# deveshjawla/MuZero.jl

Hardware: AMD Instinct MI355X
Metric: self-play MCTS node-expansions/sec + train steps/sec, TicTacToe FC net, 1-8 GPU (higher is better)
Workload: dtype f32; 1 GPU; TicTacToe FC (params.jl hyper), 512 games/GPU x 50 sims/move (configs[1]); games_per_gpu=512, sims_per_move=50, global_games=512, parallelism=games sharded x1

## Files before the change

muzero.jl_amd/csrc/mz_small.hip:

```cpp
#include "mz_mlp_device.h"
#include "mz_tree_device.h"

#include "mz_small_params.h"
#include "mz_replay_device.h"
#include "mz_learner_device.h"

#ifdef MZ_STAMPS
#define SM_STAMP(i)                                                              \
    do {                                                                         \
        if (threadIdx.x == 0) {                                                  \
            unsigned long long t_ = __builtin_amdgcn_s_memtime();                \
            st_acc[i] += t_ - st_last; st_last = t_;                             \
        }                                                                        \
    } while (0)
#define W_STAMP0() unsigned long long w_t0_ = __builtin_amdgcn_s_memtime()
#define W_STAMP(k) do { w_acc[k] += __builtin_amdgcn_s_memtime() - w_t0_; } while (0)
#else
#define SM_STAMP(i) do {} while (0)
#define W_STAMP0() do {} while (0)
#define W_STAMP(k) do {} while (0)
#endif

__device__ __forceinline__ int sm_slot_row(int tid) {
    return (tid >> 8) * 64 + ((tid >> 6) & 3) * 16 + (tid & 15);
}

template <int J>
__device__ __forceinline__ void fmac_bcast(float& acc, float x, float w) {
    asm volatile("v_fmac_f32_dpp %0, %1, %2 row_newbcast:%3 row_mask:0xf bank_mask:0xf"
                 : "+v"(acc) : "v"(x), "v"(w), "i"(J));
}

#define SM_F2(j, wj)                                                                              \
    "v_fmac_f32_dpp %0, %2, " wj " row_newbcast:" #j " row_mask:0xf bank_mask:0xf\n\t"            \
    "v_fmac_f32_dpp %1, %3, " wj " row_newbcast:" #j " row_mask:0xf bank_mask:0xf\n\t"

template <int T, int J = 0>
__device__ __forceinline__ void sm_chain(const float (&w)[16], const float (&x)[T], float (&acc)[T]) {
    if constexpr (T == 2 && J == 0) {
        asm volatile("s_nop 1\n\t"
                     SM_F2(0, "%4") SM_F2(1, "%5") SM_F2(2, "%6") SM_F2(3, "%7")
                     SM_F2(4, "%8") SM_F2(5, "%9") SM_F2(6, "%10") SM_F2(7, "%11")
                     SM_F2(8, "%12") SM_F2(9, "%13") SM_F2(10, "%14") SM_F2(11, "%15")
                     SM_F2(12, "%16") SM_F2(13, "%17") SM_F2(14, "%18") SM_F2(15, "%19")
                     : "+v"(acc[0]), "+v"(acc[1])
                     : "v"(x[0]), "v"(x[1]), "v"(w[0]), "v"(w[1]), "v"(w[2]), "v"(w[3]), "v"(w[4]), "v"(w[5]),
                       "v"(w[6]), "v"(w[7]), "v"(w[8]), "v"(w[9]), "v"(w[10]), "v"(w[11]), "v"(w[12]), "v"(w[13]),
                       "v"(w[14]), "v"(w[15]));
    } else if constexpr (J < 16) {
#pragma unroll
        for (int g = 0; g < T; ++g) fmac_bcast<J>(acc[g], x[g], w[J]);
        sm_chain<T, J + 1>(w, x, acc);
    }
}

struct SmFusedIn {
    const float* hid; const int* leaf_e; const int* leaf_a; const float* aval;
    int NN, H, plane, x_pred, x_dyn;
};

template <int T>
__device__ __forceinline__ int sm_xoff(int4 R) {
    const int q = (threadIdx.x >> 4) & 3, i = threadIdx.x & 15;
    return (R.x + ((int)__umul24((unsigned)q, (unsigned)R.y) + i) * T) * 4;
}

template <int T, int FI = 0, int BNM = 1>
__device__ __forceinline__ int4 sm_stage(const float (&w)[16], int4 R, int& xo, const int4* rec_next, float* lds,
                                         const SmFusedIn* fi = nullptr, const float2* bnp = nullptr) {
    const int q = (threadIdx.x >> 4) & 3;
    const float* xp = reinterpret_cast<const float*>(reinterpret_cast<const char*>(lds) + xo);
    float x[T];
    if constexpr (FI != 0) {
        const int k = (int)__umul24((unsigned)q, (unsigned)R.y) + (int)(threadIdx.x & 15);
        const bool pred = R.x == fi->x_pred, dyn = R.x == fi->x_dyn;
#pragma unroll
        for (int g = 0; g < T; ++g) {
            float hv, av;
            if constexpr (FI == 1) {
                const float* hp = fi->hid + ((size_t)g * fi->NN + fi->leaf_e[g]) * fi->H;
                hv = k < fi->H ? hp[k] : 0.0f;
                av = fi->aval[fi->leaf_a[g]];
            } else {
                hv = k < fi->H ? fi->hid[k * T + g] : 0.0f;
                av = fi->aval[g * fi->NN];
            }
            x[g] = pred ? hv : dyn ? (k < fi->H ? hv * 2.0f : k < fi->H + fi->plane ? av : 0.0f) : xp[g];
        }
    } else if constexpr (T == 1) {
        x[0] = xp[0];
    } else if constexpr (T == 2) {
        const float2 v = *reinterpret_cast<const float2*>(xp);
        x[0] = v.x; x[1] = v.y;
    } else {
        const float4 v = *reinterpret_cast<const float4*>(xp);
        x[0] = v.x; x[1] = v.y; x[2] = v.z; x[3] = v.w;
    }
    const int4 Rn = *rec_next;
    float acc[T];
#pragma unroll
    for (int g = 0; g < T; ++g) acc[g] = 0.0f;
    sm_chain<T>(w, x, acc);
#pragma unroll
    for (int g = 0; g < T; ++g) {
        const auto s1 = __builtin_amdgcn_permlane16_swap(__builtin_bit_cast(unsigned, acc[g]),
                                                         __builtin_bit_cast(unsigned, acc[g]), false, false);
        const float t = __builtin_bit_cast(float, (unsigned)s1[0]) + __builtin_bit_cast(float, (unsigned)s1[1]);
        const auto s2 = __builtin_amdgcn_permlane32_swap(__builtin_bit_cast(unsigned, t),
                                                         __builtin_bit_cast(unsigned, t), false, false);
        acc[g] = __builtin_bit_cast(float, (unsigned)s2[0]) + __builtin_bit_cast(float, (unsigned)s2[1]);
    }
    if (q < T && R.z >= 0) {
        float v = acc[0];
#pragma unroll
        for (int g = 1; g < T; ++g) v = q == g ? acc[g] : v;
        const int o = R.z & 0x1fffffff;
        float d = v + __int_as_float(R.w);
        if constexpr (BNM != 0)
            if ((R.z >> 29) & 1) { const float2 gb = *bnp; d = mz_bn_apply(d, gb.x, gb.y); }
        lds[o + q] = (R.z >> 30) != 0 ? mz_relu(d) : d;
    }
    xo = sm_xoff<T>(Rn);
    asm volatile("" : "+v"(xo));
    __syncthreads();
    return Rn;
}

template <int T, int NMAX, int FI, int OFF, int BNM, int K = 0>
__device__ __forceinline__ void sm_run_k(int n, const float (&wr)[NMAX][16], int4 R, int xo, const int4* rec,
                                         float* lds, const SmFusedIn* fi, const float2* bnp) {
    if constexpr (K + OFF < NMAX) {
        if (K < n) {
            const float2* bk = bnp + K * (SM_SLOTS * 64);
            const int4 Rn = K == 0 && FI != 0
                ? sm_stage<T, FI, BNM>(wr[K + OFF], R, xo, rec + (K + 1) * (SM_SLOTS * 64), lds, fi, bk)
                : sm_stage<T, 0, BNM>(wr[K + OFF], R, xo, rec + (K + 1) * (SM_SLOTS * 64), lds, nullptr, bk);
            sm_run_k<T, NMAX, FI, OFF, BNM, K + 1>(n, wr, Rn, xo, rec, lds, fi, bnp);
        }
    }
}

template <int T, int NMAX, int FI = 0, int OFF = 0, int BNM = 1>
__device__ __forceinline__ void sm_run(int n, const float (&wr)[NMAX][16], const int4* rec, float* lds,
                                       const SmFusedIn* fi, const float2* bnp) {
    const int4 R0 = rec[0];
    sm_run_k<T, NMAX, FI, OFF, BNM>(n, wr, R0, sm_xoff<T>(R0), rec, lds, fi, bnp);
}

template <int NMAX, int DST = 0>
__device__ __forceinline__ void sm_load(int k0, int k1, const float* W, float (&wr)[NMAX][16], const uint32_t* nzm,
                                        const float4* zero16) {
    const int tid = threadIdx.x, sl = tid >> 8, t = tid & 255, q = (tid >> 4) & 3;
    const int w = __builtin_amdgcn_readfirstlane(tid >> 6);
    uint32_t mk[NMAX - DST];
#pragma unroll
    for (int k = 0; k < NMAX - DST; ++k) mk[k] = nzm[w * SM_NZM_ST + k];
#pragma unroll
    for (int k = 0; k < NMAX - DST; ++k) {
        if (k >= k0 && k < k1) {
            const float4* src = reinterpret_cast<const float4*>(W + (((size_t)k * SM_SLOTS + sl) * 4) * 1024) + t;
            const uint32_t m = mk[k] >> (4 * q);
#pragma unroll
            for (int i = 0; i < 4; ++i) {
                const float4 v = *((m >> i) & 1u ? src + i * 256 : zero16);
                wr[k + DST][4 * i] = v.x; wr[k + DST][4 * i + 1] = v.y; wr[k + DST][4 * i + 2] = v.z;
                wr[k + DST][4 * i + 3] = v.w;
            }
        }
    }
}

template <int T, int BNM>
__device__ __forceinline__ void small_body(const SmallParams& P) {
#ifdef MZ_STAMPS
    unsigned long long st_acc[8] = {0, 0, 0, 0, 0, 0, 0, 0};
    unsigned long long st_last = __builtin_amdgcn_s_memtime();
    unsigned long long w_acc[3] = {0, 0, 0};
#endif
    extern __shared__ __attribute__((aligned(16))) float smem[];
    const int A = P.A, S = P.S, H = P.H;
    const int E = (S + 1) * A, NN = S + 1;
    const int PS = 2 * (S + 2);
    const int nrec = P.n_sim + P.n_root;
    float* act = smem;
    int* rec = reinterpret_cast<int*>(act + P.act_total);
    float* hid = reinterpret_cast<float*>(rec + (nrec + 1) * SM_REC_INTS);
    int* si = reinterpret_cast<int*>(hid + ((size_t)T * NN * H + 3) / 4 * 4);
    uint32_t* sg_legal = reinterpret_cast<uint32_t*>(si);
    int* sg_root_tp = si + 16;
    int* sg_rootN = si + 32;
    float* sg_rootW = reinterpret_cast<float*>(si + 48);
    float* sg_mmin = reinterpret_cast<float*>(si + 64);
    float* sg_mmax = reinterpret_cast<float*>(si + 80);
    int* sg_leaf_e = si + 96;
    int* sg_leaf_a = si + 112;
    int* sg_vtp = si + 128;
    int* sg_depth = si + 144;
    float* sg_stage = reinterpret_cast<float*>(si + 160);
    float* sg_noise = reinterpret_cast<float*>(si + 232);
    int* sg_path = si + 296;
    double* l_pbc = reinterpret_cast<double*>(si + 296 + (T * PS + 3) / 4 * 4);
    double* l_sqrt = l_pbc + (S + 2);
    float* l_aval = reinterpret_cast<float*>(l_sqrt + (S + 2));
    double* l_pbterm = reinterpret_cast<double*>(l_aval + MZ_MAX_ACTIONS);
    char* lds_tree = reinterpret_cast<char*>(l_pbterm + pbterm_count(S));
    uint2* c_cache = reinterpret_cast<uint2*>(lds_tree + (size_t)T * P.tree_game_bytes);
    uint2* c_lvl = c_cache + T * NN;
    int* c_nN = reinterpret_cast<int*>(c_lvl + T * (S + 2));
    int4* c_hdr = reinterpret_cast<int4*>(reinterpret_cast<char*>(smem) +
                                          ((reinterpret_cast<char*>(c_nN + T * NN) - reinterpret_cast<char*>(smem) + 15) & ~15));
    float2* c_mmx = reinterpret_cast<float2*>(c_hdr + 4);
    int* c_skip = reinterpret_cast<int*>(c_mmx + 4);
    const bool sel_ballot = NN <= 64;
    const int NNS = sel_ballot ? NN : 0;
    uint4* c_stat = reinterpret_cast<uint4*>(c_skip + 4);
    float2* bnl = reinterpret_cast<float2*>(c_stat + T * NNS);

    const int tid = threadIdx.x;
    const int g = tid >> 4, a = tid & 15, lane = tid & 63;
    const int tile0 = blockIdx.x * T;
    const bool tree_thread = tid < 16 * T;
    const int gg = tile0 + g;
    const bool active = tree_thread && gg < P.G;
    const uint32_t gid = P.game_offset + (uint32_t)gg;
    int* path = sg_path + (tree_thread ? g : 0) * PS;
    TreeView tree = tree_view(lds_tree + (size_t)(tree_thread ? g : 0) * P.tree_game_bytes, E, NN);
    const int4* rec_sim = reinterpret_cast<const int4*>(rec) + sm_slot_row(tid);
    const int4* rec_root = rec_sim + P.n_sim * (SM_SLOTS * 64);
    const float2* bn_sim = bnl + sm_slot_row(tid);
    const float2* bn_root = bn_sim + P.n_sim * (SM_SLOTS * 64);

    float wr[SM_MAX_SIM][16];
    sm_load<SM_MAX_SIM>(0, P.n_root, P.w_root, wr, P.nzm + P.n_sim, P.zero16);
    sm_load<SM_MAX_SIM>(P.n_root, P.n_sim, P.w_sim, wr, P.nzm, P.zero16);
    for (int i = tid; i < P.act_total; i += SM_THREADS) act[i] = 0.0f;
    for (int i = tid; i < S + 2; i += SM_THREADS) { l_pbc[i] = P.pbc_tab[i]; l_sqrt[i] = P.sqrt_tab[i]; }
    if (tid < A) l_aval[tid] = P.aval_tab[tid];
    for (int i = tid; i < (int)pbterm_count(S); i += SM_THREADS) l_pbterm[i] = P.pbterm[i];
    for (int i = tid; i < nrec * SM_REC_INTS; i += SM_THREADS) rec[i] = P.rec[i];
    __syncthreads();
    for (int i = tid; i < nrec * SM_SLOTS * 64; i += SM_THREADS)
        rec[4 * i + 3] = __float_as_int(P.bias[i]);
    if (P.bn)
        for (int i = tid; i < nrec * SM_SLOTS * 64; i += SM_THREADS)
            bnl[i] = make_float2(P.bias[nrec * SM_SLOTS * 64 + i], P.bias[2 * nrec * SM_SLOTS * 64 + i]);
    for (int i = tid; i < T * P.obs_feat; i += SM_THREADS) {
        const int gl = i / P.obs_feat, k = i - gl * P.obs_feat;
        const int ggl = tile0 + gl;
        act[P.x_rep + k * T + gl] = ggl < P.G ? P.obs[(size_t)ggl * P.obs_feat + k] : 0.0f;
    }
    for (int i = tid; i < T * NN; i += SM_THREADS) c_cache[i] = make_uint2(0u, 0u);
    if (tid < 4) { c_hdr[tid] = make_int4(0, -1, 1, 0); c_mmx[tid] = make_float2(0.0f, 0.0f); c_skip[tid] = 0; }
    if (tid < T && sel_ballot) c_stat[tid * NNS] = node_static(0, 0, 0, 1ull);
    int ver = 1;
    if (tree_thread && a == 0) {
        uint32_t m = 0;
        if (active)
            for (int b = 0; b < A; ++b) if (P.legal[(size_t)gg * A + b]) m |= 1u << b;
        sg_legal[g] = m;
        sg_root_tp[g] = active ? P.to_play[gg] : 1;
        sg_rootN[g] = 0; sg_rootW[g] = 0.0f;
        sg_mmin[g] = INFINITY; sg_mmax[g] = -INFINITY;
        sg_leaf_e[g] = 0; sg_leaf_a[g] = 0; sg_vtp[g] = 1; sg_depth[g] = 0;
    }
    __syncthreads();

    if (P.exploration && active)
        sg_noise[16 * g + a] = root_noise_lane(sg_legal[g], a, A, P.seed, gid, P.rng_step, P.dirichlet_alpha,
                                               sg_stage + 16 * g);
    sm_run<T, SM_MAX_SIM, 0, 0, BNM>(P.n_root, wr, rec_root, act, nullptr, bn_root);
    for (int i = tid; i < T * H; i += SM_THREADS) {
        const int gl = i / H, k = i - gl * H;
        const float h = act[P.h_out + k * T + gl];
        hid[(size_t)gl * NN * H + k] = h;
        act[P.x_pred + k * T + gl] = h;
    }
    sm_load<SM_MAX_SIM>(0, P.n_root < P.n_sim ? P.n_root : P.n_sim, P.w_sim, wr, P.nzm, P.zero16);
    __syncthreads();
    sm_run<T, SM_MAX_SIM, 0, 0, BNM>(P.n_sim, wr, rec_sim, act, nullptr, bn_sim);

    const uint32_t legal = tree_thread ? sg_legal[g] : 0u;
    if (tree_thread) {
        const float prior = double_softmax_prior(a < A ? act[P.p_out + a * T + g] : 0.0f, a, A, legal,
                                                 sg_stage + 16 * g);
        if (active) {
            init_edges(tree, 0, a, A, prior);
            if (a == 0) { tree.nr[0] = 0.0f; tree.ntp[0] = (int8_t)sg_root_tp[g]; }
        }
    }
    __syncthreads();
    if (P.exploration && active && a < A && ((legal >> a) & 1u))
        tree.p(a) = tree.p(a) * (1.0f - P.exploration_eps) + sg_noise[16 * g + a] * P.exploration_eps;
    __syncthreads();
    SM_STAMP(0);

    const SmFusedIn fin{hid, sg_leaf_e, sg_leaf_a, l_aval, NN, H, P.plane, P.x_pred, P.x_dyn};
    int n_fast = 0;
    for (int s = 0; s < S; ++s) {
        if (tid < 64 * T) {
            const int w = __builtin_amdgcn_readfirstlane(tid >> 6);
            if (tile0 + w < P.G) {
                const TreeView tw = tree_view(lds_tree + (size_t)w * P.tree_game_bytes, E, NN);
                int* pw = sg_path + w * PS;
                const uint2* cw = c_cache + w * NN;
                const uint32_t verw = (uint32_t)c_hdr[w].z;
                const int rtp = sg_root_tp[w];
                SelectOut so{0, 0, 1, 0};
                int D, e0;
                uint32_t npc0;
                bool found = false;
                if (sel_ballot) {
                    found = select_path_ballot(tw, cw, c_stat + w * NNS, verw, pw, s + 1, s + 1, rtp, lane, A,
                                               P.players, so, D, e0, npc0);
                } else {
                    D = c_skip[w];
                    e0 = D > 0 ? pw[2 * D + 1] : 0;
                    npc0 = D > 0 ? tw.nc(pw[2 * D]) : 0u;
                }
                if (!found && lane < 16) {
                    so = select_path_cached(tw, cw, verw, pw, sg_rootN[w], rtp, sg_legal[w], sg_mmin[w], sg_mmax[w],
                                            lane, lane, A, P.players, l_pbterm, P.seed,
                                            P.game_offset + (uint32_t)(tile0 + w), P.rng_step, s, nullptr, nullptr, D,
                                            e0, npc0);
                    if (sel_ballot && lane == 0) {
                        const uint4 ps = c_stat[w * NNS + so.leaf_e];
                        c_stat[w * NNS + s + 1] = node_static(so.leaf_e, so.depth, so.leaf_a,
                                                              ((uint64_t)ps.y | ((uint64_t)ps.z << 32)) | (1ull << (s + 1)));
                    }
                }
                if (lane == 0) { sg_leaf_e[w] = so.leaf_e; sg_leaf_a[w] = so.leaf_a; sg_vtp[w] = so.vtp; sg_depth[w] = so.depth; }
                n_fast += found ? 1 : 0;
            }
            __builtin_amdgcn_wave_barrier();
            SM_STAMP(1);
        }
        __syncthreads();
#ifdef MZ_STAMPS
        if (threadIdx.x == 0) {
            int md = 0;
            for (int gl = 0; gl < T; ++gl) md = md > sg_depth[gl] ? md : sg_depth[gl];
            st_acc[7] += (unsigned long long)md;
        }
#endif
        SM_STAMP(2);
        sm_run<T, SM_MAX_SIM, 1, 0, BNM>(P.n_sim, wr, rec_sim, act, &fin, bn_sim);
        SM_STAMP(3);
        const int e_new = s + 1;
        if (tid < 64) {
            if (active) {
                const int tl = sg_vtp[g];
                const int depth = sg_depth[g];
                const BackupPre bpre = backup_preload(tree, path, depth, a);
                const bool odd = (a & 1) != 0;
                const float ro = mz_post_act(odd ? P.r_act : P.v_act, act[(odd ? P.r_out : P.v_out) + g]);
                const float val = __builtin_bit_cast(float, __builtin_amdgcn_update_dpp(
                    0, __builtin_bit_cast(int, ro), 0x00, 0xF, 0xF, false));
                const float rew = __builtin_bit_cast(float, __builtin_amdgcn_update_dpp(
                    0, __builtin_bit_cast(int, ro), 0x55, 0xF, 0xF, false));
#ifdef MZ_STAMPS
                if (threadIdx.x == 0) asm volatile("" :: "v"(val), "v"(rew));
#endif
                SM_STAMP(5);
                W_STAMP0();
                if (a == 0) {
                    const int li = sg_leaf_e[g] * A + sg_leaf_a[g];
                    tree.nc(li) = (tree.nc(li) & 0xffffu) | ((uint32_t)(e_new + 1) << 16);
                    tree.nr[e_new] = rew;
                    tree.ntp[e_new] = (int8_t)tl;
                    path[2 * depth + 1] = e_new;
                }
                __builtin_amdgcn_wave_barrier();
                int rN = sg_rootN[g];
                float rW = sg_rootW[g], mmin = sg_mmin[g], mmax = sg_mmax[g];
                const uint32_t omin = __float_as_uint(mmin), omax = __float_as_uint(mmax);
                if (P.players == 2)
                    backup_path_pre(tree, path, bpre, depth, val, rew, e_new, tl, P.discount, rN, rW, sg_root_tp[g],
                                    mmin, mmax, a, c_lvl + g * (S + 2), c_nN + g * NN);
                else
                    backup_path(tree, path, depth, val, tl, A, P.players, P.discount, rN, rW, sg_root_tp[g], mmin,
                                mmax, a, c_lvl + g * (S + 2), c_nN + g * NN);
                const bool moved = __float_as_uint(mmin) != omin || __float_as_uint(mmax) != omax;
                ver += moved ? 1 : 0;
                if (a == 0) {
                    sg_rootN[g] = rN; sg_rootW[g] = rW; sg_mmin[g] = mmin; sg_mmax[g] = mmax;
                    c_hdr[g] = make_int4(moved ? 1 : 0, depth, ver, (int)legal);
                    c_mmx[g] = make_float2(mmin, mmax);
                    c_skip[g] = moved ? 0 : depth;
                }
                W_STAMP(0);
            }
        } else if (tid >= 128 && tid < 128 + 16 * T) {
            W_STAMP0();
            const int g2 = (tid - 128) >> 4;
            const bool active2 = tile0 + g2 < P.G;
            TreeView tree2 = tree_view(lds_tree + (size_t)g2 * P.tree_game_bytes, E, NN);
            const float prior = double_softmax_prior(a < A ? act[P.p_out + a * T + g2] : 0.0f, a, A, sg_legal[g2],
                                                     sg_stage + 16 * g2);
            if (active2) init_edges(tree2, e_new, a, A, prior);
            W_STAMP(1);
        } else if (tid >= 192) {
            W_STAMP0();
            for (int i = tid - 192; i < T * H; i += SM_THREADS - 192) {
                const int gl = i / H, k = i - gl * H;
                hid[((size_t)gl * NN + e_new) * H + k] = act[P.h_out + k * T + gl];
                if (tile0 + gl < P.G) {
                    float* hp = hid + ((size_t)gl * NN + sg_leaf_e[gl]) * H + k;
                    *hp = *hp * 2.0f;
                }
            }
            W_STAMP(2);
        }
        __syncthreads();
        SM_STAMP(4);
        if (s + 1 < S) {
            const int r = tid >> 4, gq = r % T, j0 = r / T;
            int4 hd = c_hdr[gq];
            float2 mm = c_mmx[gq];
            uint2 l0 = c_lvl[gq * (S + 2) + j0];
            int n0 = c_nN[gq * NN + j0];
            asm volatile("" : "+v"(hd.x), "+v"(hd.y), "+v"(hd.z), "+v"(hd.w), "+v"(mm.x), "+v"(mm.y), "+v"(l0.x),
                              "+v"(l0.y), "+v"(n0));
            const bool full = hd.x != 0;
            const int n = full ? s + 2 : hd.y + 1;
            const bool lgl = a < A && (((uint32_t)hd.w >> a) & 1u);
            const TreeView tq = tree_view(lds_tree + (size_t)gq * P.tree_game_bytes, E, NN);
            uint2* cq = c_cache + gq * NN;
            const int* pq = sg_path + gq * PS;
            const int pe0 = !full && j0 < hd.y ? pq[2 * (j0 + 1)] : 0;
            if (j0 < n) {
                const int ch = cache_row(tq, cq, (uint32_t)hd.z, full ? j0 : (int)l0.x, full ? n0 : (int)l0.y, lgl,
                                         a, A, mm.x, mm.y, l_pbterm, lane);
                if (!full && a == 0 && (j0 >= hd.y || ch != pe0 - (int)l0.x * A)) atomicMin(c_skip + gq, j0);
            }
            for (int j = j0 + SM_THREADS / 16 / T; j < n; j += SM_THREADS / 16 / T) {
                int slot, Np;
                if (full) { slot = j; Np = c_nN[gq * NN + j]; }
                else { const uint2 l = c_lvl[gq * (S + 2) + j]; slot = (int)l.x; Np = (int)l.y; }
                const int ch = cache_row(tq, cq, (uint32_t)hd.z, slot, Np, lgl, a, A, mm.x, mm.y, l_pbterm, lane);
                if (!full && a == 0 && (j >= hd.y || ch != pq[2 * (j + 1)] - slot * A)) atomicMin(c_skip + gq, j);
            }
            __syncthreads();
            SM_STAMP(6);
        }
    }
    __syncthreads();

    if (active) {
        const bool lg = a < A && ((legal >> a) & 1u);
        const int Nc = lg ? (int)(tree.nc(a) & 0xffffu) : 0;
        const int sum = g16_isum(Nc);
        if (a < A) P.child_visits[(size_t)gg * A + a] = lg ? (float)((double)Nc / (double)sum) : 0.0f;
        const uint32_t r = mz_rng_u32(P.seed, MZ_RNG_ACTION, gid, P.rng_step, 0);
        const int act = select_action_dev<16>(Nc, legal, A, P.temp_g ? P.temp_g[gg] : P.temperature, r);
        if (a == 0) {
            const int rN = sg_rootN[g];
            P.root_value[gg] = rN == 0 ? 0.0f : sg_rootW[g] / (float)rN;
            P.action_out[gg] = act + 1;
        }
        if (P.dump_tree) {
            TreeView dst = tree_view(P.tree + (size_t)gg * P.tree_game_bytes, E, NN);
            dump_tree(tree, dst, E, NN, a);
        }
    }
    if (P.sel_stats && tid < 64 * T && lane == 0 && tile0 + (tid >> 6) < P.G) {
        P.sel_stats[2 * (tile0 + (tid >> 6))] = n_fast;
        P.sel_stats[2 * (tile0 + (tid >> 6)) + 1] = S - n_fast;
    }
#ifdef MZ_STAMPS
    SM_STAMP(6);
    if (threadIdx.x == 0 && P.stamps)
        for (int i = 0; i < 8; ++i) P.stamps[blockIdx.x * 8 + i] = st_acc[i];
    if (P.stamps && (threadIdx.x == 0 || threadIdx.x == 128 || threadIdx.x == 192)) {
        const int k = threadIdx.x == 0 ? 0 : threadIdx.x == 128 ? 1 : 2;
        P.stamps[(gridDim.x + blockIdx.x) * 8 + k] = w_acc[k];
    }
#endif
}

extern "C" __global__ __launch_bounds__(SM_THREADS, 1) void mz_search_small1(SmallParams P) { small_body<1, 0>(P); }
extern "C" __global__ __launch_bounds__(SM_THREADS, 1) void mz_search_small2(SmallParams P) { small_body<2, 0>(P); }
extern "C" __global__ __launch_bounds__(SM_THREADS, 1) void mz_search_small4(SmallParams P) { small_body<4, 0>(P); }
extern "C" __global__ __launch_bounds__(SM_THREADS, 1) void mz_search_small1_bn(SmallParams P) { small_body<1, 1>(P); }
extern "C" __global__ __launch_bounds__(SM_THREADS, 1) void mz_search_small2_bn(SmallParams P) { small_body<2, 1>(P); }
extern "C" __global__ __launch_bounds__(SM_THREADS, 1) void mz_search_small4_bn(SmallParams P) { small_body<4, 1>(P); }

struct SmIO {
    const float* obs; const float* actions; float* pv; float* pp; float* pr;
    const float* w_sim; const float* w_root; const float* bias;
};
__device__ __forceinline__ SmIO sm_io(const SmallUnrollParams& P) {
    return SmIO{P.obs, P.actions, P.pv, P.pp, P.pr, P.w_sim, P.w_root, P.bias};
}

template <int T, int BNM>
__device__ __forceinline__ void unroll_body(const SmallUnrollParams& P, int lb, const SmIO& io) {
#ifdef MZ_STAMPS
    unsigned long long st_acc[8] = {0, 0, 0, 0, 0, 0, 0, 0};
    unsigned long long st_last = __builtin_amdgcn_s_memtime();
#endif
    extern __shared__ __attribute__((aligned(16))) float smem[];
    const int K = P.K, A = P.A, H = P.H;
    const int nrec = P.n_sim + P.n_root;
    float* act = smem;
    int* rec = reinterpret_cast<int*>(act + P.act_total);
    float* aval = reinterpret_cast<float*>(rec + (nrec + 1) * SM_REC_INTS);
    float2* bnl = reinterpret_cast<float2*>(aval + 64);
    const int tid = threadIdx.x;
    const int tile0 = lb * T;
    const int o_gl = tid / (A + 2), o_c = tid - o_gl * (A + 2);
    const int nri = nrec * SM_SLOTS * 64;
    constexpr int RPT = ((SM_MAX_SIM + SM_MAX_ROOT) * SM_SLOTS * 64 + SM_THREADS - 1) / SM_THREADS;
    const bool sample_first = !P.pf_hdr && P.sample;
    if (sample_first && (tid >> 6) < T && tile0 + (tid >> 6) < P.B) rp_sample_one(P.rp, tile0 + (tid >> 6), tid & 63);
    if (sample_first) { __threadfence_block(); __syncthreads(); }
    long long hd[4] = {0, 0, 0, 0}, cnt0 = 0;
    if (P.pf_hdr) { hd[0] = P.pf_hdr[0]; hd[1] = P.pf_hdr[1]; hd[2] = P.pf_hdr[2]; hd[3] = P.pf_hdr[3]; cnt0 = P.rp.counters[0]; }
    int rx[RPT], ry[RPT], rz[RPT];
    float bv[RPT];
#pragma unroll
    for (int u = 0; u < RPT; ++u) {
        const int i = tid + u * SM_THREADS;
        const int ic = i < nri ? i : 0;
        const int4 r = reinterpret_cast<const int4*>(P.rec)[ic];
        rx[u] = r.x; ry[u] = r.y; rz[u] = r.z;
        bv[u] = io.bias[ic];
    }
    const int o_i = tid / P.obs_feat, o_k = tid - o_i * P.obs_feat;
    const int a_i = tid / (K + 1), a_k = tid - a_i * (K + 1);
    const bool o_in = tid < T * P.obs_feat && tile0 + o_i < P.B, a_in = tid < T * (K + 1) && tile0 + a_i < P.B;
    float ov = o_in ? io.obs[(size_t)(tile0 + o_i) * P.obs_feat + o_k] : 0.0f;
    float av = a_in ? io.actions[(size_t)(tile0 + a_i) * (K + 1) + a_k] : 0.0f;
    float wr[SM_MAX_SIM][16];
    constexpr int RO = SM_MAX_SIM - SM_MAX_ROOT;
    sm_load<SM_MAX_SIM, RO>(0, P.n_root, io.w_root, wr, P.nzm + P.n_sim, P.zero16);
    sm_load<SM_MAX_SIM>(0, RO < P.n_sim ? RO : P.n_sim, io.w_sim, wr, P.nzm, P.zero16);
    sm_load<SM_MAX_SIM>(RO + P.n_root, P.n_sim, io.w_sim, wr, P.nzm, P.zero16);
    const bool have = P.pf_hdr && hd[0] == P.pf_epoch && hd[1] == cnt0 && hd[2] == (long long)P.rp.step &&
                      hd[3] == (long long)P.B;
    if (P.pf_hdr && P.sample && !have) {
        if ((tid >> 6) < T && tile0 + (tid >> 6) < P.B) rp_sample_one(P.rp, tile0 + (tid >> 6), tid & 63);
        __threadfence_block();
        __syncthreads();
        ov = o_in ? io.obs[(size_t)(tile0 + o_i) * P.obs_feat + o_k] : 0.0f;
        av = a_in ? io.actions[(size_t)(tile0 + a_i) * (K + 1) + a_k] : 0.0f;
    }
    for (int i = tid; i < P.act_total; i += SM_THREADS) act[i] = 0.0f;
#pragma unroll
    for (int u = 0; u < RPT; ++u) {
        const int i = tid + u * SM_THREADS;
        if (i < nri) reinterpret_cast<int4*>(rec)[i] = make_int4(rx[u], ry[u], rz[u], __float_as_int(bv[u]));
    }
    if (tid < SM_REC_INTS / 4) reinterpret_cast<int4*>(rec)[nri + tid] = make_int4(0, 0, -1, 0);
    if (P.bn)
        for (int i = tid; i < nri; i += SM_THREADS) bnl[i] = make_float2(io.bias[nri + i], io.bias[2 * nri + i]);
    __syncthreads();
    if (o_in) act[P.x_rep + o_k * T + o_i] = ov;
    if (a_in) aval[a_i * (K + 1) + a_k] = av / (float)A;
    __syncthreads();
    SM_STAMP(0);
    const int4* rec_sim = reinterpret_cast<const int4*>(rec) + sm_slot_row(tid);
    const int4* rec_root = rec_sim + P.n_sim * (SM_SLOTS * 64);
    const float2* bn_sim = bnl + sm_slot_row(tid);
    const float2* bn_root = bn_sim + P.n_sim * (SM_SLOTS * 64);
    sm_run<T, SM_MAX_SIM, 0, RO, BNM>(P.n_root, wr, rec_root, act, nullptr, bn_root);
    SM_STAMP(1);
    sm_load<SM_MAX_SIM>(RO, RO + P.n_root < P.n_sim ? RO + P.n_root : P.n_sim, io.w_sim, wr, P.nzm, P.zero16);
    SM_STAMP(2);
    for (int i = 1; i <= K; ++i) {
        const SmFusedIn fin{act + P.h_out, nullptr, nullptr, aval + (i - 1), K + 1, H, P.plane, P.x_pred, P.x_dyn};
        SM_STAMP(3);
        sm_run<T, SM_MAX_SIM, 2, 0, BNM>(P.n_sim, wr, rec_sim, act, &fin, bn_sim);
        SM_STAMP(4);
        if (tid < T * (A + 2) && tile0 + o_gl < P.B) {
            const int gl = o_gl, c = o_c;
            const int bb = tile0 + gl;
            float x;
            float* dst;
            float* dst0 = nullptr;
            if (c < A) {
                x = act[P.p_out + c * T + gl];
                dst = io.pp + ((size_t)bb * (K + 1) + i) * A + c;
                if (i == 1) dst0 = io.pp + ((size_t)bb * (K + 1)) * A + c;
            } else if (c == A) {
                x = act[P.v_out + gl];
                dst = io.pv + (size_t)bb * (K + 1) + i;
                if (i == 1) dst0 = io.pv + (size_t)bb * (K + 1);
            } else {
                x = act[P.r_out + gl];
                dst = io.pr + (size_t)bb * (K + 1) + i;
                if (i == 1) io.pr[(size_t)bb * (K + 1)] = 0.0f;
            }
            *dst = x;
            if (dst0) *dst0 = x;
        }
        SM_STAMP(5);
    }
#ifdef MZ_STAMPS
    if (threadIdx.x == 0 && P.stamps)
        for (int i = 0; i < 8; ++i) P.stamps[lb * 8 + i] = st_acc[i];
#endif
}

extern "C" __global__ __launch_bounds__(SM_THREADS, 1) void mz_unroll_small1(SmallUnrollParams P) { unroll_body<1, 0>(P, blockIdx.x, sm_io(P)); }
extern "C" __global__ __launch_bounds__(SM_THREADS, 1) void mz_unroll_small2(SmallUnrollParams P) { unroll_body<2, 0>(P, blockIdx.x, sm_io(P)); }
extern "C" __global__ __launch_bounds__(SM_THREADS, 1) void mz_unroll_small1_bn(SmallUnrollParams P) { unroll_body<1, 1>(P, blockIdx.x, sm_io(P)); }
extern "C" __global__ __launch_bounds__(SM_THREADS, 1) void mz_unroll_small2_bn(SmallUnrollParams P) { unroll_body<2, 1>(P, blockIdx.x, sm_io(P)); }

template <int T, int BNM>
__device__ __forceinline__ void learn_body(const SmallUnrollParams& P, const LearnParams& L) {
    __shared__ float stg[SM_THREADS];
    __shared__ double red[SM_THREADS];
    const int tid = threadIdx.x;
    const int K1 = P.K + 1, n = P.B * K1;
    float* vsq = L.terms;
    float* cet = L.terms + n;
#ifdef MZ_STAMPS
    const unsigned long long t_start = __builtin_amdgcn_s_memtime();
#endif
    const int lb = (int)blockIdx.x;
    if (lb < L.nU) {
        unroll_body<T, BNM>(P, lb, sm_io(P));
#ifdef MZ_STAMPS
        const unsigned long long t_unroll = __builtin_amdgcn_s_memtime();
#endif
        __syncthreads();
        const int g16 = tid >> 4, a = tid & 15, gl = g16 / K1, k = g16 - gl * K1;
        const int b = lb * T + gl;
        if (gl < T && b < P.B)
            lg_step_terms<16>(b * K1 + k, a, P.A, P.v_act, P.r_act, P.pv, P.pp, P.pr, L.tv, L.tp, vsq, cet,
                              stg + (tid & ~15));
#ifdef MZ_STAMPS
        if (tid == 0 && P.stamps) {
            P.stamps[lb * 8 + 6] = t_unroll - t_start;
            P.stamps[lb * 8 + 7] = __builtin_amdgcn_s_memtime() - t_unroll;
        }
#endif
    } else if (lb >= L.nU + LEARN_L2_GROUPS) {
        const int b = (lb - L.nU - LEARN_L2_GROUPS) * (SM_THREADS / 64) + (tid >> 6);
        if (b < L.pfq.B && L.pf_nb > 0) rp_sample_one(L.pfq, b, tid & 63);
        if (lb == L.nU + LEARN_L2_GROUPS && L.pf_nb > 0 && tid == 0) {
            L.pf_hdr_next[0] = L.pf_epoch;
            L.pf_hdr_next[1] = L.pfq.counters[0];
            L.pf_hdr_next[2] = (long long)L.pfq.step;
            L.pf_hdr_next[3] = (long long)L.pfq.B;
        }
    } else {
        const int half = tid >> 8, t256 = tid & (MZ_THREADS - 1);
        for (int pass = 0; pass < LEARN_L2_PASSES; ++pass) {
            const int vb = (pass * LEARN_L2_GROUPS + lb - L.nU) * SM_SLOTS + half;
            const bool vin = vb < 3 * MZ_L2_BLOCKS;
            const int net = vb / MZ_L2_BLOCKS, blk = vb % MZ_L2_BLOCKS;
            red[tid] = vin ? lg_l2_slice(net, blk, t256, L.netoff, L.flat, nullptr, L.ad) : 0.0;
            __syncthreads();
            for (int o = MZ_THREADS / 2; o > 0; o >>= 1) {
                if (t256 < o) red[tid] += red[tid + o];
                __syncthreads();
            }
            if (t256 == 0 && vin)
                __hip_atomic_store(L.part + net * MZ_L2_BLOCKS + blk, red[tid], __ATOMIC_RELAXED,
                                   __HIP_MEMORY_SCOPE_AGENT);
            __syncthreads();
        }
    }
    lg_fold(P.B, P.K, vsq, cet, L.gscale, nullptr, L.part, L.counter, L.out);
}

extern "C" __global__ __launch_bounds__(SM_THREADS, 1) void mz_learn_small1(SmallUnrollParams P, LearnParams L) {
    learn_body<1, 0>(P, L);
}
extern "C" __global__ __launch_bounds__(SM_THREADS, 1) void mz_learn_small2(SmallUnrollParams P, LearnParams L) {
    learn_body<2, 0>(P, L);
}
extern "C" __global__ __launch_bounds__(SM_THREADS, 1) void mz_learn_small1_bn(SmallUnrollParams P, LearnParams L) {
    learn_body<1, 1>(P, L);
}
extern "C" __global__ __launch_bounds__(SM_THREADS, 1) void mz_learn_small2_bn(SmallUnrollParams P, LearnParams L) {
    learn_body<2, 1>(P, L);
}


template <bool CAP, bool HELP>
__device__ __forceinline__ void chain_param(const ChainParams& C, size_t p, double* rd, float* hx,
                                            const double (*sbp)[MZ_MULTI_MAX]) {
    const int L = C.L;
    float x = C.flat[p], m = C.M[p], v = C.V[p];
    const int it = C.inv_tile[p], is = C.inv_small[p];
    const bool sbank = C.bank_w != nullptr, tbank = C.tbank_w != nullptr;
    for (int i = 0; i < L; ++i) {
        if constexpr (HELP) __hip_atomic_store(hx + (size_t)i * C.hx_n, x, __ATOMIC_RELAXED, __HIP_MEMORY_SCOPE_AGENT);
        else rd[i * MZ_THREADS] += (double)x * (double)x;
        if (sbank) mz_scatter(x, is, C.bank_w + i * C.bws, C.bank_b + i * C.bbs);
        if (tbank) mz_scatter(x, it, C.tbank_w + i * C.tws, C.tbank_b + i * C.tbs);
        if (C.fbank) C.fbank[i * C.fstride + p] = x;
        x = adam_2theta(x, m, v, sbp[0][i], sbp[1][i], sbp[2][i]);
        if (C.theta) C.theta[i * C.nflat + p] = x;
        if constexpr (CAP) {
            if (i == C.cap_i[0]) {
                C.cap_dst[0][p] = x;
                if (C.cap_img[0]) {
                    mz_scatter(x, it, C.cap_img[0], C.cap_img[1]);
                    mz_scatter(x, is, C.cap_img[2], C.cap_img[3]);
                }
            }
            if (i == C.cap_i[1]) C.cap_dst[1][p] = x;
        }
    }
    C.flat[p] = x; C.M[p] = m; C.V[p] = v;
    mz_scatter(x, it, C.Wp, C.Bp);
    mz_scatter(x, is, C.smw, C.smb);
}

template <bool CAP>
__device__ __forceinline__ void chain_slice(const ChainParams& C, int net, int sb, double (*red)[MZ_THREADS],
                                            double (*sbp)[MZ_MULTI_MAX]) {
    const int tid = threadIdx.x;
    const size_t off = C.netoff[net], cnt = C.netoff[3 + net];
    const size_t stride = (size_t)MZ_L2_BLOCKS * MZ_THREADS;
    for (size_t e = (size_t)sb * MZ_THREADS + tid; e < cnt; e += stride)
        chain_param<CAP, false>(C, off + e, &red[0][tid], nullptr, sbp);
}

__device__ __forceinline__ void chain_tree(double (*red)[MZ_THREADS], int L, double* part) {
    const int tid = threadIdx.x;
    for (int o = MZ_THREADS / 2; o > 0; o >>= 1) {
        for (int x = tid; x < o * L; x += MZ_THREADS) {
            const int i = x / o, j = x - i * o;
            red[i][j] += red[i][j + o];
        }
        __syncthreads();
    }
    if (tid < L) part[(size_t)tid * 3 * MZ_L2_BLOCKS] = red[tid][0];
}

__device__ __forceinline__ int chain_npart(const ChainParams& C, int net, int sb) {
    return 1 + (C.nh[net] > sb ? (C.nh[net] - 1 - sb) / MZ_L2_BLOCKS + 1 : 0);
}

__device__ __forceinline__ void chain_arrive(const ChainParams& C, int net, int sb, double (*red)[MZ_THREADS],
                                             int* last) {
    const int tid = threadIdx.x, L = C.L;
    asm volatile("s_waitcnt vmcnt(0)" ::: "memory");
    __syncthreads();
    if (tid == 0) {
        const unsigned long long np = (unsigned long long)chain_npart(C, net, sb);
        const unsigned long long old = __hip_atomic_fetch_add(C.hcnt + net * MZ_L2_BLOCKS + sb, 1ull,
                                                              __ATOMIC_ACQ_REL, __HIP_MEMORY_SCOPE_AGENT);
        *last = (old + 1) % np == 0;
    }
    __syncthreads();
    if (!*last) return;
    const size_t cnt = C.netoff[3 + net], stride = (size_t)MZ_L2_BLOCKS * MZ_THREADS;
    const auto rs = __builtin_amdgcn_make_buffer_rsrc(C.hx, (short)0, (int)(MZ_MULTI_MAX * C.hx_n * 4), 0x00020000);
    for (int i = 0; i < L; ++i) red[i][tid] = 0.0;
    for (size_t e = (size_t)sb * MZ_THREADS + tid; e < cnt; e += stride) {
        const int b0 = (int)((C.hoff[net] + e) * 4);
        float xv[MZ_MULTI_MAX];
#pragma unroll
        for (int i = 0; i < MZ_MULTI_MAX; ++i)
            xv[i] = __uint_as_float(__builtin_amdgcn_raw_buffer_load_b32(rs, b0 + (int)(i * C.hx_n * 4), 0, 16));
#pragma unroll
        for (int i = 0; i < MZ_MULTI_MAX; ++i)
            if (i < L) red[i][tid] += (double)xv[i] * (double)xv[i];
    }
    __syncthreads();
    chain_tree(red, L, C.part + net * MZ_L2_BLOCKS + sb);
}

extern "C" __global__ __launch_bounds__(MZ_THREADS) void mz_learn_chain(ChainParams C) {
    __shared__ double red[MZ_MULTI_MAX][MZ_THREADS];
    __shared__ double sbp[3][MZ_MULTI_MAX];
    __shared__ int last;
    const int tid = threadIdx.x, nht = C.nh[0] + C.nh[1] + C.nh[2];
    const int blk = (int)blockIdx.x - nht;
    constexpr int NSL = 3 * MZ_L2_BLOCKS;
    const size_t stride = (size_t)MZ_L2_BLOCKS * MZ_THREADS;
    const int L = C.L;
    const bool cap = C.cap_i[0] >= 0 || C.cap_i[1] >= 0;
    if (blk >= NSL) {
        const int q = (blk - NSL) * (MZ_THREADS / 64) + (tid >> 6);
        if (q >= L * C.B) return;
        const int i = q / C.B, b = q - i * C.B;
        RpSampleParams Q = C.q;
        Q.step += (uint32_t)i;
        Q.obs += i * C.s_obs; Q.actions += i * C.s_k1; Q.tv += i * C.s_k1; Q.tr += i * C.s_k1;
        Q.tpol += i * C.s_tp; Q.gscale += (size_t)i * C.B; Q.index += (size_t)i * 2 * C.B;
        rp_sample_one(Q, b, tid & 63);
        return;
    }
    if (tid < MZ_MULTI_MAX) { sbp[0][tid] = C.bp1[tid]; sbp[1][tid] = C.bp2[tid]; sbp[2][tid] = C.eta[tid]; }
    __syncthreads();
    int net, sb;
    size_t e;
    if (blk < 0) {
        int hb = (int)blockIdx.x;
        net = 0;
        while (hb >= C.nh[net]) hb -= C.nh[net++];
        e = stride + (size_t)hb * MZ_THREADS + tid;
        sb = hb % MZ_L2_BLOCKS;
    } else {
        net = blk / MZ_L2_BLOCKS;
        sb = blk - net * MZ_L2_BLOCKS;
        e = (size_t)sb * MZ_THREADS + tid;
    }
    if (blk < 0 || chain_npart(C, net, sb) > 1) {
        if (e < C.netoff[3 + net]) {
            float* hx = C.hx + C.hoff[net] + e;
            if (cap) chain_param<true, true>(C, C.netoff[net] + e, nullptr, hx, sbp);
            else chain_param<false, true>(C, C.netoff[net] + e, nullptr, hx, sbp);
        }
        chain_arrive(C, net, sb, red, &last);
        return;
    }
    for (int i = 0; i < L; ++i) red[i][tid] = 0.0;
    __syncthreads();
    if (cap) chain_slice<true>(C, net, sb, red, sbp);
    else chain_slice<false>(C, net, sb, red, sbp);
    __syncthreads();
    chain_tree(red, L, C.part + blk);
}

template <int T, int BNM>
__device__ __forceinline__ void learn_multi_body(const SmallUnrollParams& P, const LearnMultiParams& M) {
    __shared__ float stg[SM_THREADS];
    const int tid = threadIdx.x, pb = (int)blockIdx.x;
    int i, lb;
    if (M.xcd) {
        const int r = pb >> 3;
        i = (pb & 7) + 8 * (r / M.nU);
        lb = r % M.nU;
    } else {
        i = pb / M.nU;
        lb = pb - i * M.nU;
    }
    if (i >= M.L) return;
    const int K1 = P.K + 1;
    if (M.sample) {
        const int w = tid >> 6, b = lb * T + w;
        if (w < T && b < P.B) {
            RpSampleParams Q = M.q;
            Q.step += (uint32_t)i;
            Q.obs += i * M.s_obs; Q.actions += i * M.s_k1; Q.tv += i * M.s_k1; Q.tr += i * M.s_k1;
            Q.tpol += i * M.s_tp; Q.gscale += (size_t)i * P.B; Q.index += (size_t)i * 2 * P.B;
            rp_sample_one(Q, b, tid & 63);
        }
        __threadfence_block();
        __syncthreads();
    }
    SmIO io;
    io.obs = M.obs + i * M.s_obs; io.actions = M.act + i * M.s_k1;
    io.pv = M.pv + i * M.s_k1; io.pp = M.pp + i * M.s_tp; io.pr = M.pr + i * M.s_k1;
    io.w_sim = M.bank_w + i * M.bws;
    io.w_root = io.w_sim + (size_t)P.n_sim * SM_SLOTS * 256 * 16;
    io.bias = M.bank_b + i * M.bbs;
    unroll_body<T, BNM>(P, lb, io);
    __syncthreads();
    float* vsq = M.terms + 2 * i * M.s_k1;
    float* cet = vsq + M.s_k1;
    const int g16 = tid >> 4, a = tid & 15, gl = g16 / K1, k = g16 - gl * K1;
    const int b = lb * T + gl;
    if (gl < T && b < P.B)
        lg_step_terms<16>(b * K1 + k, a, P.A, P.v_act, P.r_act, io.pv, io.pp, io.pr, M.tv + i * M.s_k1,
                          M.tp + i * M.s_tp, vsq, cet, stg + (tid & ~15));
    lg_fold(P.B, P.K, vsq, cet, M.gs + (size_t)i * P.B, nullptr, M.part + (size_t)i * 3 * MZ_L2_BLOCKS,
            M.counter + i * MZ_MULTI_CNT_STRIDE, M.out_last && i == M.L - 1 ? M.out_last : M.out + 8 * i,
            (unsigned)M.nU);
}

extern "C" __global__ __launch_bounds__(SM_THREADS, 1) void mz_learn_multi1(SmallUnrollParams P, LearnMultiParams M) {
    learn_multi_body<1, 0>(P, M);
}
extern "C" __global__ __launch_bounds__(SM_THREADS, 1) void mz_learn_multi2(SmallUnrollParams P, LearnMultiParams M) {
    learn_multi_body<2, 0>(P, M);
}
extern "C" __global__ __launch_bounds__(SM_THREADS, 1) void mz_learn_multi4(SmallUnrollParams P, LearnMultiParams M) {
    learn_multi_body<4, 0>(P, M);
}
extern "C" __global__ __launch_bounds__(SM_THREADS, 1) void mz_learn_multi4_bn(SmallUnrollParams P, LearnMultiParams M) {
    learn_multi_body<4, 1>(P, M);
}
extern "C" __global__ __launch_bounds__(SM_THREADS, 1) void mz_learn_multi1_bn(SmallUnrollParams P, LearnMultiParams M) {
    learn_multi_body<1, 1>(P, M);
}
extern "C" __global__ __launch_bounds__(SM_THREADS, 1) void mz_learn_multi2_bn(SmallUnrollParams P, LearnMultiParams M) {
    learn_multi_body<2, 1>(P, M);
}
```

Measured before the change: 94.13 million node-expansions/s.

## Overlap kernel prologue setup with weight loads and specialize noise wave

Restructures the search kernel prologue. Global loads for rec, bias, pbterm and obs are issued into registers before the weight image is loaded, then written to LDS afterwards. One dedicated wave does legal-mask, root state and Dirichlet-noise init in parallel with the others, and the LDS zeroing now skips the obs region. Waves without root weights skip the root stage and only match its barriers, and simulation-stage weights are reloaded a fixed number of stages ahead instead of all reloaded up front. This aims to hide global-memory latency in the per-move prologue, at the cost of more register pressure and more complex per-wave control flow.

```diff
diff --git a/muzero.jl_amd/csrc/mz_small.hip b/muzero.jl_amd/csrc/mz_small.hip
--- a/muzero.jl_amd/csrc/mz_small.hip
+++ b/muzero.jl_amd/csrc/mz_small.hip
@@ -15,10 +15,16 @@
     } while (0)
 #define W_STAMP0() unsigned long long w_t0_ = __builtin_amdgcn_s_memtime()
 #define W_STAMP(k) do { w_acc[k] += __builtin_amdgcn_s_memtime() - w_t0_; } while (0)
+#define P_MARK(i)                                                                \
+    do {                                                                         \
+        if ((threadIdx.x & 255) == 0)                                            \
+            p_mark[i] = (__builtin_amdgcn_s_memtime() - p_t0) & 0x1fffffull;     \
+    } while (0)
 #else
 #define SM_STAMP(i) do {} while (0)
 #define W_STAMP0() do {} while (0)
 #define W_STAMP(k) do {} while (0)
+#define P_MARK(i) do {} while (0)
 #endif
 
 __device__ __forceinline__ int sm_slot_row(int tid) {
@@ -170,12 +176,49 @@
     }
 }
 
+__device__ __forceinline__ void sm_load_set(float (&w)[16], const float* W, int stage, uint32_t mask,
+                                            const float4* zero16) {
+    const int tid = threadIdx.x, sl = tid >> 8, t = tid & 255, q = (tid >> 4) & 3;
+    const float4* src = reinterpret_cast<const float4*>(W + (((size_t)stage * SM_SLOTS + sl) * 4) * 1024) + t;
+    const uint32_t m = mask >> (4 * q);
+#pragma unroll
+    for (int i = 0; i < 4; ++i) {
+        const float4 v = *((m >> i) & 1u ? src + i * 256 : zero16);
+        w[4 * i] = v.x; w[4 * i + 1] = v.y; w[4 * i + 2] = v.z; w[4 * i + 3] = v.w;
+    }
+    __builtin_amdgcn_sched_barrier(0);
+}
+
+template <int T, int BNM, int LEAD, int K = 0>
+__device__ __forceinline__ void sm_run_reload_k(int n, float (&wr)[SM_MAX_SIM][16], int4 R, int xo, const int4* rec,
+                                                float* lds, const float2* bnp, bool reload, const float* W,
+                                                const uint32_t (&mk)[SM_MAX_SIM], const float4* zero16) {
+    if constexpr (K < SM_MAX_SIM) {
+        if (K < n) {
+            if constexpr (K + LEAD < SM_MAX_SIM)
+                if (reload) sm_load_set(wr[K + LEAD], W, K + LEAD, mk[K + LEAD], zero16);
+            const int4 Rn = sm_stage<T, 0, BNM>(wr[K], R, xo, rec + (K + 1) * (SM_SLOTS * 64), lds, nullptr,
+                                                bnp + K * (SM_SLOTS * 64));
+            sm_run_reload_k<T, BNM, LEAD, K + 1>(n, wr, Rn, xo, rec, lds, bnp, reload, W, mk, zero16);
+        }
+    }
+}
+template <int T, int BNM, int LEAD>
+__device__ __forceinline__ void sm_run_reload(int n, float (&wr)[SM_MAX_SIM][16], const int4* rec, float* lds,
+                                              const float2* bnp, bool reload, const float* W,
+                                              const uint32_t (&mk)[SM_MAX_SIM], const float4* zero16) {
+    const int4 R0 = rec[0];
+    sm_run_reload_k<T, BNM, LEAD>(n, wr, R0, sm_xoff<T>(R0), rec, lds, bnp, reload, W, mk, zero16);
+}
+
 template <int T, int BNM>
 __device__ __forceinline__ void small_body(const SmallParams& P) {
 #ifdef MZ_STAMPS
     unsigned long long st_acc[8] = {0, 0, 0, 0, 0, 0, 0, 0};
     unsigned long long st_last = __builtin_amdgcn_s_memtime();
     unsigned long long w_acc[3] = {0, 0, 0};
+    const unsigned long long p_t0 = st_last;
+    unsigned long long p_mark[7] = {0, 0, 0, 0, 0, 0, 0};
 #endif
     extern __shared__ __attribute__((aligned(16))) float smem[];
     const int A = P.A, S = P.S, H = P.H;
@@ -230,54 +273,140 @@
     const float2* bn_sim = bnl + sm_slot_row(tid);
     const float2* bn_root = bn_sim + P.n_sim * (SM_SLOTS * 64);
 
+    constexpr int NW = 4 * (SM_SLOTS - 1);
+    static_assert(NW >= 4, "the noise wave is not one of the first slot's");
+    constexpr int CT = SM_THREADS - 64;
+    const int ci = tid < 64 * NW ? tid : tid - 64;
+    constexpr int RO = SM_MAX_SIM - SM_MAX_ROOT;
     float wr[SM_MAX_SIM][16];
-    sm_load<SM_MAX_SIM>(0, P.n_root, P.w_root, wr, P.nzm + P.n_sim, P.zero16);
-    sm_load<SM_MAX_SIM>(P.n_root, P.n_sim, P.w_sim, wr, P.nzm, P.zero16);
-    for (int i = tid; i < P.act_total; i += SM_THREADS) act[i] = 0.0f;
-    for (int i = tid; i < S + 2; i += SM_THREADS) { l_pbc[i] = P.pbc_tab[i]; l_sqrt[i] = P.sqrt_tab[i]; }
-    if (tid < A) l_aval[tid] = P.aval_tab[tid];
-    for (int i = tid; i < (int)pbterm_count(S); i += SM_THREADS) l_pbterm[i] = P.pbterm[i];
-    for (int i = tid; i < nrec * SM_REC_INTS; i += SM_THREADS) rec[i] = P.rec[i];
-    __syncthreads();
-    for (int i = tid; i < nrec * SM_SLOTS * 64; i += SM_THREADS)
-        rec[4 * i + 3] = __float_as_int(P.bias[i]);
-    if (P.bn)
-        for (int i = tid; i < nrec * SM_SLOTS * 64; i += SM_THREADS)
-            bnl[i] = make_float2(P.bias[nrec * SM_SLOTS * 64 + i], P.bias[2 * nrec * SM_SLOTS * 64 + i]);
-    for (int i = tid; i < T * P.obs_feat; i += SM_THREADS) {
-        const int gl = i / P.obs_feat, k = i - gl * P.obs_feat;
-        const int ggl = tile0 + gl;
-        act[P.x_rep + k * T + gl] = ggl < P.G ? P.obs[(size_t)ggl * P.obs_feat + k] : 0.0f;
-    }
-    for (int i = tid; i < T * NN; i += SM_THREADS) c_cache[i] = make_uint2(0u, 0u);
-    if (tid < 4) { c_hdr[tid] = make_int4(0, -1, 1, 0); c_mmx[tid] = make_float2(0.0f, 0.0f); c_skip[tid] = 0; }
-    if (tid < T && sel_ballot) c_stat[tid * NNS] = node_static(0, 0, 0, 1ull);
+    const int wv = __builtin_amdgcn_readfirstlane(tid >> 6);
+    uint32_t mk_sim[SM_MAX_SIM], mk_root[SM_MAX_ROOT];
+    uint32_t any_root = 0;
+#pragma unroll
+    for (int k = 0; k < SM_MAX_SIM; ++k) mk_sim[k] = k < P.n_sim ? P.nzm[wv * SM_NZM_ST + k] : 0u;
+#pragma unroll
+    for (int k = 0; k < SM_MAX_ROOT; ++k) {
+        mk_root[k] = k < P.n_root ? P.nzm[wv * SM_NZM_ST + P.n_sim + k] : 0u;
+        any_root |= mk_root[k];
+    }
+    const bool root_wave = any_root != 0;
+    auto image = [&]() __attribute__((always_inline)) {
+#pragma unroll
+        for (int j = 0; j < SM_MAX_SIM; ++j) {
+            const int k = j < SM_MAX_ROOT ? j + RO : j - SM_MAX_ROOT;
+            const bool rs = root_wave && k >= RO;
+            sm_load_set(wr[k], rs ? P.w_root : P.w_sim, rs ? k - RO : k,
+                        rs ? mk_root[k >= RO ? k - RO : 0] : mk_sim[k], P.zero16);
+        }
+        P_MARK(0);
+    };
     int ver = 1;
-    if (tree_thread && a == 0) {
-        uint32_t m = 0;
-        if (active)
-            for (int b = 0; b < A; ++b) if (P.legal[(size_t)gg * A + b]) m |= 1u << b;
-        sg_legal[g] = m;
-        sg_root_tp[g] = active ? P.to_play[gg] : 1;
-        sg_rootN[g] = 0; sg_rootW[g] = 0.0f;
-        sg_mmin[g] = INFINITY; sg_mmax[g] = -INFINITY;
-        sg_leaf_e[g] = 0; sg_leaf_a[g] = 0; sg_vtp[g] = 1; sg_depth[g] = 0;
-    }
-    __syncthreads();
-
-    if (P.exploration && active)
-        sg_noise[16 * g + a] = root_noise_lane(sg_legal[g], a, A, P.seed, gid, P.rng_step, P.dirichlet_alpha,
-                                               sg_stage + 16 * g);
-    sm_run<T, SM_MAX_SIM, 0, 0, BNM>(P.n_root, wr, rec_root, act, nullptr, bn_root);
+    if (wv != NW) {
+        const int nri = nrec * SM_SLOTS * 64;
+        constexpr int RPT = ((SM_MAX_SIM + SM_MAX_ROOT) * SM_SLOTS * 64 + CT - 1) / CT;
+        constexpr int PBT = 2;
+        const int npb = (int)pbterm_count(S), npb2 = npb >> 1;
+        for (int i = ci + PBT * CT; i < npb2; i += CT)
+            reinterpret_cast<double2*>(l_pbterm)[i] = reinterpret_cast<const double2*>(P.pbterm)[i];
+        for (int i = ci + CT; i < S + 2; i += CT) { l_pbc[i] = P.pbc_tab[i]; l_sqrt[i] = P.sqrt_tab[i]; }
+        int rx[RPT], ry[RPT], rz[RPT];
+        float bv[RPT], bg[RPT], bb[RPT];
+#pragma unroll
+        for (int u = 0; u < RPT; ++u) {
+            const int i = ci + u * CT;
+            const int ic = i < nri ? i : 0;
+            const int4 r = reinterpret_cast<const int4*>(P.rec)[ic];
+            rx[u] = r.x; ry[u] = r.y; rz[u] = r.z;
+            bv[u] = P.bias[ic];
+            if constexpr (BNM != 0) {
+                bg[u] = P.bias[P.bn ? nri + ic : 0];
+                bb[u] = P.bias[P.bn ? 2 * nri + ic : 0];
+            }
+        }
+        double pbx[PBT], pby[PBT];
+#pragma unroll
+        for (int u = 0; u < PBT; ++u) {
+            const int i = ci + u * CT;
+            const double2 v = reinterpret_cast<const double2*>(P.pbterm)[i < npb2 ? i : 0];
+            pbx[u] = v.x; pby[u] = v.y;
+        }
+        const double pbl = P.pbterm[npb - 1];
+        const double pcv = P.pbc_tab[ci < S + 2 ? ci : 0], sqv = P.sqrt_tab[ci < S + 2 ? ci : 0];
+        const float avv = P.aval_tab[tid < A ? tid : 0];
+        const int o_gl = tid / P.obs_feat, o_k = tid - o_gl * P.obs_feat;
+        const bool o_it = tid < T * P.obs_feat, o_in = o_it && tile0 + o_gl < P.G;
+        const float ov = P.obs[o_in ? (size_t)(tile0 + o_gl) * P.obs_feat + o_k : 0];
+        image();
+        for (int i = ci; i < P.act_total; i += CT)
+            if (i < P.x_rep || i >= P.x_rep + T * P.obs_feat) act[i] = 0.0f;
+        if (o_it) act[P.x_rep + o_k * T + o_gl] = o_in ? ov : 0.0f;
+#pragma unroll
+        for (int u = 0; u < RPT; ++u) {
+            const int i = ci + u * CT;
+            if (i < nri) {
+                reinterpret_cast<int4*>(rec)[i] = make_int4(rx[u], ry[u], rz[u], __float_as_int(bv[u]));
+                if constexpr (BNM != 0)
+                    if (P.bn) bnl[i] = make_float2(bg[u], bb[u]);
+            }
+        }
+#pragma unroll
+        for (int u = 0; u < PBT; ++u) {
+            const int i = ci + u * CT;
+            if (i < npb2) reinterpret_cast<double2*>(l_pbterm)[i] = make_double2(pbx[u], pby[u]);
+        }
+        if (tid == 0 && (npb & 1)) l_pbterm[npb - 1] = pbl;
+        if (ci < S + 2) { l_pbc[ci] = pcv; l_sqrt[ci] = sqv; }
+        if (tid < A) l_aval[tid] = avv;
+        for (int i = ci; i < T * NN; i += CT) c_cache[i] = make_uint2(0u, 0u);
+        if (tid < 4) { c_hdr[tid] = make_int4(0, -1, 1, 0); c_mmx[tid] = make_float2(0.0f, 0.0f); c_skip[tid] = 0; }
+        if (tid < T && sel_ballot) c_stat[tid * NNS] = node_static(0, 0, 0, 1ull);
+        P_MARK(1);
+        P_MARK(2);
+    } else {
+        const int n_g = (tid - 64 * NW) >> 4, n_gg = tile0 + n_g;
+        const bool n_active = n_g < T && n_gg < P.G;
+        if (n_g < T) {
+            const uint8_t lgb = P.legal[n_active && a < A ? (size_t)n_gg * A + a : 0];
+            const int tpv = P.to_play[n_active ? n_gg : 0];
+            const uint32_t lmask = g16_or(n_active && a < A && lgb ? 1u << a : 0u);
+            if (a == 0) {
+                sg_legal[n_g] = lmask;
+                sg_root_tp[n_g] = n_active ? tpv : 1;
+                sg_rootN[n_g] = 0; sg_rootW[n_g] = 0.0f;
+                sg_mmin[n_g] = INFINITY; sg_mmax[n_g] = -INFINITY;
+                sg_leaf_e[n_g] = 0; sg_leaf_a[n_g] = 0; sg_vtp[n_g] = 1; sg_depth[n_g] = 0;
+            }
+            if (P.exploration && n_active)
+                sg_noise[16 * n_g + a] = root_noise_lane(lmask, a, A, P.seed, P.game_offset + (uint32_t)n_gg,
+                                                         P.rng_step, P.dirichlet_alpha, sg_stage + 16 * n_g);
+        }
+        P_MARK(2);
+        if (root_wave) image();
+    }
+    __syncthreads();
+    if (root_wave) {
+        sm_run<T, SM_MAX_SIM, 0, RO, BNM>(P.n_root, wr, rec_root, act, nullptr, bn_root);
+    } else {
+        if (wv == NW) image();
+        for (int k = 0; k < P.n_root; ++k) __syncthreads();
+    }
+    P_MARK(3);
+    __builtin_amdgcn_s_waitcnt(0x0f70);
+    if (root_wave) {
+#pragma unroll
+        for (int k = RO; k < RO + 2; ++k) sm_load_set(wr[k], P.w_sim, k, mk_sim[k], P.zero16);
+    }
+    P_MARK(4);
     for (int i = tid; i < T * H; i += SM_THREADS) {
         const int gl = i / H, k = i - gl * H;
         const float h = act[P.h_out + k * T + gl];
         hid[(size_t)gl * NN * H + k] = h;
         act[P.x_pred + k * T + gl] = h;
     }
-    sm_load<SM_MAX_SIM>(0, P.n_root < P.n_sim ? P.n_root : P.n_sim, P.w_sim, wr, P.nzm, P.zero16);
-    __syncthreads();
-    sm_run<T, SM_MAX_SIM, 0, 0, BNM>(P.n_sim, wr, rec_sim, act, nullptr, bn_sim);
+    __syncthreads();
+    sm_run_reload<T, BNM, RO + 2>(P.n_sim, wr, rec_sim, act, bn_sim, root_wave, P.w_sim, mk_sim, P.zero16);
+    __builtin_amdgcn_s_waitcnt(0x0f70);
+    P_MARK(5);
 
     const uint32_t legal = tree_thread ? sg_legal[g] : 0u;
     if (tree_thread) {
@@ -292,6 +421,7 @@
     if (P.exploration && active && a < A && ((legal >> a) & 1u))
         tree.p(a) = tree.p(a) * (1.0f - P.exploration_eps) + sg_noise[16 * g + a] * P.exploration_eps;
     __syncthreads();
+    P_MARK(6);
     SM_STAMP(0);
 
     const SmFusedIn fin{hid, sg_leaf_e, sg_leaf_a, l_aval, NN, H, P.plane, P.x_pred, P.x_dyn};
@@ -474,6 +604,12 @@
         const int k = threadIdx.x == 0 ? 0 : threadIdx.x == 128 ? 1 : 2;
         P.stamps[(gridDim.x + blockIdx.x) * 8 + k] = w_acc[k];
     }
+    if (P.stamps && (threadIdx.x & 255) == 0) {
+        unsigned long long* pw = P.stamps + (gridDim.x + blockIdx.x) * 8 + (threadIdx.x == 0 ? 3 : 6);
+        pw[0] = p_mark[0] | p_mark[1] << 21 | p_mark[2] << 42;
+        pw[1] = p_mark[3] | p_mark[4] << 21 | p_mark[5] << 42;
+        if (threadIdx.x == 0) pw[2] = p_mark[6];
+    }
 #endif
 }
 
```

Result: faster. 96.35 million node-expansions/s, median of 6 (+2.4%).
